# fabiocarrara/neural-ode-features

Measured on AMD Instinct MI355X. Metric: images/sec (fwd+adjoint) CIFAR-10 ODE-ResNet bs=128 at 1/2/4/8 GPU, higher is better.
Workload: dtype f32

## Files before the change

### include/node_hip.h

```cpp
#ifndef NODE_HIP_H
#define NODE_HIP_H

#include <stddef.h>
#include <stdint.h>

#ifdef __cplusplus
extern "C" {
#endif

#define NODE_ABI_VERSION 6

enum { NODE_METHOD_DOPRI5 = 0, NODE_METHOD_RK4 = 1 };

enum {
  NODE_OK = 0,
  NODE_ERR_NULL = -1,
  NODE_ERR_SHAPE = -2,
  NODE_ERR_UNSUPPORTED = -3,
  NODE_ERR_WORKSPACE = -4,
  NODE_ERR_MAX_STEPS = -5,
  NODE_ERR_NONFINITE = -6,
  NODE_ERR_DT_UNDERFLOW = -7,
  NODE_ERR_HIP = -8,
  NODE_ERR_ARG = -9
// ... 217 lines not shown
  const float* b1_c2_w;
  const float* b1_ds_w;
  const float* b2_n1_w;
  const float* b2_n1_b;
  const float* b2_c1_w;
  const float* b2_n2_w;
  const float* b2_n2_b;
  const float* b2_c2_w;
  const float* b2_ds_w;
} node_stem_params;
typedef struct node_stem_grads {
  float* conv0_w; float* conv0_b;
  float* b1_n1_w; float* b1_n1_b; float* b1_c1_w; float* b1_n2_w; float* b1_n2_b; float* b1_c2_w; float* b1_ds_w;
  float* b2_n1_w; float* b2_n1_b; float* b2_c1_w; float* b2_n2_w; float* b2_n2_b; float* b2_c2_w; float* b2_ds_w;
} node_stem_grads;
size_t node_stem_workspace_bytes(const node_stem_shape* shape);
int node_stem_fwd(const node_stem_shape* shape, const node_stem_params* params, const float* x, float* out,
                  void* ws, size_t ws_bytes, void* stream);
int node_stem_bwd(const node_stem_shape* shape, const node_stem_params* params, const float* x, const float* grad_out,
                  const node_stem_grads* grads, void* ws, size_t ws_bytes, void* stream);
int node_stem_bwd_dx(const node_stem_shape* shape, const node_stem_params* params, const float* x, const float* grad_out,
                     const node_stem_grads* grads, float* d_x, void* ws, size_t ws_bytes, void* stream);
size_t node_stem_conv0_dgrad_workspace_bytes(const node_stem_shape* shape);
int node_stem_conv0_dgrad(const node_stem_shape* shape, const float* w0, const float* dy, float* d_x,
                          void* ws, size_t ws_bytes, void* stream);

typedef struct node_conv_geom {
  int32_t n, cin, cout, x_h, x_w, k, stride, pad;
} node_conv_geom;
size_t node_stem_conv_workspace_bytes(const node_conv_geom* g);
int node_stem_conv(const node_conv_geom* g, int what, const float* x, const float* w, const float* dy, float* result,
                   void* ws, size_t ws_bytes, void* stream);

typedef struct node_trunk_shape {
  int32_t n, channels, h, w, blocks;
  float eps;
} node_trunk_shape;
typedef struct node_trunk_block {
  const float* n1_w;
  const float* n1_b;
  const float* c1_w;
  const float* n2_w;
  const float* n2_b;
  const float* c2_w;
} node_trunk_block;
typedef struct node_trunk_block_grads {
  float* n1_w; float* n1_b; float* c1_w; float* n2_w; float* n2_b; float* c2_w;
} node_trunk_block_grads;
size_t node_trunk_workspace_bytes(const node_trunk_shape* shape, int keep_for_backward);
int node_trunk_fwd(const node_trunk_shape* shape, const node_trunk_block* blocks, const float* x, float* out, float* taps,
                   int keep_for_backward, void* ws, size_t ws_bytes, void* stream);
int node_trunk_bwd(const node_trunk_shape* shape, const node_trunk_block* blocks, const float* grad_out,
                   const node_trunk_block_grads* grads, float* d_x, void* ws, size_t ws_bytes, void* stream);

size_t node_retrieval_workspace_bytes(int nq, int nd, int d);
int node_retrieval_ap(int nq, int nd, int d, const float* q, const float* x, const int32_t* q_labels, const int32_t* x_labels,
                      int k, double* ap, double* ap_k, void* ws, size_t ws_bytes, void* stream);
int node_rank_ap(int nq, int nd, const float* scores, const int32_t* q_labels, const int32_t* x_labels, int k, double* ap,
                 double* ap_k, void* ws, size_t ws_bytes, void* stream);

typedef struct { int32_t fold; int32_t cls; float c; } node_svm_problem;
typedef struct { int32_t iterations; int32_t converged; double grad_ratio; } node_svm_result;
size_t node_svm_workspace_bytes(int n, int d, int p);
int node_svm_fit(int n, int d, int p, const float* x, const int32_t* labels, const int32_t* row_fold,
                 const node_svm_problem* problems, double eps, int max_iter, float* weights, node_svm_result* results, void* ws,
                 size_t ws_bytes, void* stream);
// ... 55 lines not shown
```

### neural-ode-features_amd/_lib.py

```python
from __future__ import annotations

import ctypes as C
import os

HERE = os.path.dirname(os.path.abspath(__file__))
LIB_PATH = os.path.join(HERE, 'csrc', 'libnode_hip.so')
LIB_DIAG_PATH = os.path.join(HERE, 'csrc', 'libnode_hip_diag.so')

NODE_ABI_VERSION = 6
METHOD_DOPRI5, METHOD_RK4 = 0, 1
METHODS = {'dopri5': METHOD_DOPRI5, 'rk4': METHOD_RK4}

ERRORS = {
    0: 'NODE_OK', -1: 'NODE_ERR_NULL', -2: 'NODE_ERR_SHAPE', -3: 'NODE_ERR_UNSUPPORTED',
    -4: 'NODE_ERR_WORKSPACE', -5: 'NODE_ERR_MAX_STEPS', -6: 'NODE_ERR_NONFINITE',
    -7: 'NODE_ERR_DT_UNDERFLOW', -8: 'NODE_ERR_HIP', -9: 'NODE_ERR_ARG',
}

EXPORTS = [
    'node_abi_version', 'node_last_error', 'node_param_count', 'node_workspace_bytes', 'node_solve_is_resident',
    'node_describe_dims',
    'node_odefunc_fwd', 'node_odefunc_vjp', 'node_solve_fwd', 'node_solve_adjoint',
    'node_backprop_workspace_bytes', 'node_solve_backprop',
    'node_head_fwd', 'node_head_bwd', 'node_gn_relu_fwd', 'node_gn_relu_bwd',
    'node_sgd_step', 'node_adam_step', 'node_profile_begin', 'node_profile_end',
    'node_conv3x3_w4_workspace_bytes', 'node_conv3x3_w4', 'node_w4_split3', 'node_w4_pair_stats',
    'node_stem_workspace_bytes', 'node_stem_fwd', 'node_stem_bwd', 'node_stem_conv_workspace_bytes', 'node_stem_conv',
    'node_stem_bwd_dx', 'node_stem_conv0_dgrad_workspace_bytes', 'node_stem_conv0_dgrad', 'node_attack_step', 'node_attack_judge',
    'node_head_loss_scratch_bytes', 'node_head_loss_fwd', 'node_head_loss_bwd',
    'node_flat_workspace_bytes', 'node_flat_begin', 'node_flat_stage', 'node_flat_scalar', 'node_flat_initial_step',
    'node_flat_finish_step', 'node_flat_status_read',
    'node_retrieval_workspace_bytes', 'node_retrieval_ap', 'node_rank_ap',
    'node_svm_workspace_bytes', 'node_svm_fit', 'node_svm_cv_score',
    'node_augment_batch',
    'node_imgconv_workspace_bytes', 'node_imgconv_fwd', 'node_imgconv_bwd',
    'node_trunk_workspace_bytes', 'node_trunk_fwd', 'node_trunk_bwd',
]


class NodeShape(C.Structure):
    _fields_ = [('n', C.c_int32), ('c', C.c_int32), ('h', C.c_int32), ('w', C.c_int32),
                ('groups', C.c_int32), ('eps', C.c_float)]


class NodeParams(C.Structure):
    _fields_ = [(k, C.c_void_p) for k in (
        'norm1_w', 'norm1_b', 'conv1_w', 'conv1_b', 'norm2_w', 'norm2_b',
        'conv2_w', 'conv2_b', 'norm3_w', 'norm3_b')]


WGRAD_KERNELS = ('W2_8', 'W2_4', 'W_8_8', 'W_16_2', 'W_4_4', 'T_8_8', 'T_16_4', 'T_7_7', 'T_4_4', 'P')
CONV_KERNELS = ('DIRECT_64', 'DIRECT_128', 'DIRECT_256', 'W1_64', 'W1_128', 'W1_256', 'W2_128')


class NodeDimsInfo(C.Structure):
    _fields_ = [(k, C.c_int32) for k in (
        'wgrad_kernel', 'conv_kernel', 'wino', 'bm', 's', 'csplit', 'mtiles', 'ntile', 'small', 'tiny', 'wino4', 'w4q',
        'wgrad_wino', 'wut', 'rb', 'nbands', 'nsplit', 'wgrad_pair')]


# ... 43 lines not shown

class NodeAdamTensor(C.Structure):
    _fields_ = [('param', C.c_void_p), ('grad', C.c_void_p), ('exp_avg', C.c_void_p), ('exp_avg_sq', C.c_void_p),
                ('step', C.c_void_p), ('n', C.c_size_t)]


STEM_PARAM_FIELDS = ('conv0_w', 'conv0_b', 'b1_n1_w', 'b1_n1_b', 'b1_c1_w', 'b1_n2_w', 'b1_n2_b', 'b1_c2_w', 'b1_ds_w',
                     'b2_n1_w', 'b2_n1_b', 'b2_c1_w', 'b2_n2_w', 'b2_n2_b', 'b2_c2_w', 'b2_ds_w')


class NodeStemShape(C.Structure):
    _fields_ = [('n', C.c_int32), ('in_ch', C.c_int32), ('h', C.c_int32), ('w', C.c_int32), ('filters', C.c_int32),
                ('eps', C.c_float)]


class NodeStemParams(C.Structure):
    _fields_ = [(k, C.c_void_p) for k in STEM_PARAM_FIELDS]


TRUNK_BLOCK_FIELDS = ('n1_w', 'n1_b', 'c1_w', 'n2_w', 'n2_b', 'c2_w')


class NodeTrunkShape(C.Structure):
    _fields_ = [('n', C.c_int32), ('channels', C.c_int32), ('h', C.c_int32), ('w', C.c_int32), ('blocks', C.c_int32),
                ('eps', C.c_float)]


class NodeTrunkBlock(C.Structure):
    _fields_ = [(k, C.c_void_p) for k in TRUNK_BLOCK_FIELDS]


class NodeConvGeom(C.Structure):
    _fields_ = [(k, C.c_int32) for k in ('n', 'cin', 'cout', 'x_h', 'x_w', 'k', 'stride', 'pad')]


REDUCE_MEAN, REDUCE_SUM = 0, 1


class NodeHeadLoss(C.Structure):
    _fields_ = [('n', C.c_int32), ('c', C.c_int32), ('classes', C.c_int32), ('reduction', C.c_int32),
                ('pooled', C.c_void_p), ('weight', C.c_void_p), ('bias', C.c_void_p), ('target', C.c_void_p),
                ('logits', C.c_void_p), ('loss', C.c_void_p), ('stat', C.c_void_p), ('scratch', C.c_void_p)]


class NodeHeadLossGrad(C.Structure):
    _fields_ = [(k, C.c_void_p) for k in ('grad_loss', 'grad_logits', 'd_logits', 'd_pooled', 'd_weight', 'd_bias')]


class NodeFlatSeg(C.Structure):
    _fields_ = [('y', C.c_void_p), ('y1', C.c_void_p), ('k', C.c_void_p * 7), ('n', C.c_size_t)]


class NodeFlatSolve(C.Structure):
    _fields_ = [('nseg', C.c_int32), ('has_scalar', C.c_int32), ('seg', NodeFlatSeg * 3), ('rtol', C.c_float), ('atol', C.c_float),
                ('tsign', C.c_float), ('n_targets', C.c_int32), ('ws', C.c_void_p), ('ws_bytes', C.c_size_t)]


class NodeFlatStatus(C.Structure):
    _fields_ = [('done', C.c_int32), ('status', C.c_int32), ('steps', C.c_int32), ('accepted', C.c_int32), ('rejected', C.c_int32),
                ('t', C.c_double), ('dt', C.c_double), ('first_dt', C.c_double), ('scalar', C.c_float)]


FLAT_F0, FLAT_PROBE = -1, -2

AUG_CROP, AUG_JITTER, AUG_FLIP, AUG_NORM = 1, 2, 4, 8

# ... 75 lines not shown
    lib.node_head_fwd.argtypes = [P(NodeShape), vp, vp, vp, vp, vp, vp, vp]
    lib.node_head_bwd.restype = i32
    lib.node_head_bwd.argtypes = [P(NodeShape), vp, vp, vp, vp, vp, vp, vp, vp, vp, vp]
    lib.node_gn_relu_fwd.restype = i32
    lib.node_gn_relu_fwd.argtypes = [P(NodeShape), vp, vp, vp, i32, vp, vp, vp]
    lib.node_gn_relu_bwd.restype = i32
    lib.node_gn_relu_bwd.argtypes = [P(NodeShape), vp, vp, vp, vp, i32, vp, vp, vp, vp, vp]
    lib.node_sgd_step.restype = i32
    lib.node_sgd_step.argtypes = [P(NodeSgdTensor), i32, f32, f32, f32, f32, vp, vp]
    lib.node_adam_step.restype = i32
    lib.node_adam_step.argtypes = [P(NodeAdamTensor), i32, f32, f32, f32, f32, f32, f32, vp, vp]
    lib.node_profile_begin.restype = i32
    lib.node_profile_begin.argtypes = []
    lib.node_profile_end.restype = i32
    lib.node_profile_end.argtypes = [P(NodeProfile)]
    lib.node_conv3x3_w4_workspace_bytes.restype = sz
    lib.node_conv3x3_w4_workspace_bytes.argtypes = [P(NodeShape)]
    lib.node_w4_pair_stats.restype = i32
    lib.node_w4_pair_stats.argtypes = [P(C.c_int32)]
    lib.node_conv3x3_w4.restype = i32
    lib.node_conv3x3_w4.argtypes = [P(NodeShape), vp, i32, vp, vp, vp, sz, vp]
    lib.node_w4_split3.restype = i32
    lib.node_w4_split3.argtypes = [vp, vp, sz, vp]
    lib.node_stem_workspace_bytes.restype = sz
    lib.node_stem_workspace_bytes.argtypes = [P(NodeStemShape)]
    lib.node_stem_fwd.restype = i32
    lib.node_stem_fwd.argtypes = [P(NodeStemShape), P(NodeStemParams), vp, vp, vp, sz, vp]
    lib.node_stem_bwd.restype = i32
    lib.node_stem_bwd.argtypes = [P(NodeStemShape), P(NodeStemParams), vp, vp, P(NodeStemParams), vp, sz, vp]
    lib.node_stem_conv_workspace_bytes.restype = sz
    lib.node_stem_conv_workspace_bytes.argtypes = [P(NodeConvGeom)]
    lib.node_stem_conv.restype = i32
    lib.node_stem_conv.argtypes = [P(NodeConvGeom), i32, vp, vp, vp, vp, vp, sz, vp]
    lib.node_stem_bwd_dx.restype = i32
    lib.node_stem_bwd_dx.argtypes = [P(NodeStemShape), P(NodeStemParams), vp, vp, P(NodeStemParams), vp, vp, sz, vp]
    lib.node_stem_conv0_dgrad_workspace_bytes.restype = sz
    lib.node_stem_conv0_dgrad_workspace_bytes.argtypes = [P(NodeStemShape)]
    lib.node_stem_conv0_dgrad.restype = i32
    lib.node_stem_conv0_dgrad.argtypes = [P(NodeStemShape), vp, vp, vp, vp, sz, vp]
    lib.node_attack_step.restype = i32
    lib.node_attack_step.argtypes = [P(NodeAttack), vp, vp, vp, vp, vp, vp]
    lib.node_attack_judge.restype = i32
    lib.node_attack_judge.argtypes = [P(NodeAttack), i32, vp, vp, vp, vp, i32, i32, P(NodeAttackRecord), vp]
    lib.node_head_loss_scratch_bytes.restype = sz
    lib.node_head_loss_scratch_bytes.argtypes = [i32]
    lib.node_head_loss_fwd.restype = i32
    lib.node_head_loss_fwd.argtypes = [P(NodeHeadLoss), vp]
    lib.node_head_loss_bwd.restype = i32
    lib.node_head_loss_bwd.argtypes = [P(NodeHeadLoss), P(NodeHeadLossGrad), vp]
    lib.node_flat_workspace_bytes.restype = sz
    lib.node_flat_workspace_bytes.argtypes = [i32]
    lib.node_flat_begin.restype = i32
    lib.node_flat_begin.argtypes = [P(NodeFlatSolve), C.c_double, P(C.c_double), C.c_double, i32, vp]
    lib.node_flat_stage.restype = i32
    lib.node_flat_stage.argtypes = [P(NodeFlatSolve), i32, i32, P(C.c_void_p), vp, vp]
    lib.node_flat_scalar.restype = i32
    lib.node_flat_scalar.argtypes = [P(NodeFlatSolve), i32, vp, f32, i32, vp]
    lib.node_flat_initial_step.restype = i32
    lib.node_flat_initial_step.argtypes = [P(NodeFlatSolve), i32, vp]
    lib.node_flat_finish_step.restype = i32
    lib.node_flat_finish_step.argtypes = [P(NodeFlatSolve), i32, vp, vp]
    lib.node_flat_status_read.restype = i32
    lib.node_flat_status_read.argtypes = [P(NodeFlatSolve), P(NodeFlatStatus), vp]
    lib.node_retrieval_workspace_bytes.restype = sz
    lib.node_retrieval_workspace_bytes.argtypes = [i32, i32, i32]
    lib.node_retrieval_ap.restype = i32
# ... 34 lines not shown
```

### neural-ode-features_amd/csrc/kernels_stem.hip

```cpp
#include "stem.h"
#include <type_traits>

namespace node {

namespace {

typedef float f32x16 __attribute__((ext_vector_type(16)));
typedef __bf16 bf16x8 __attribute__((ext_vector_type(8)));
typedef __bf16 bf16x2 __attribute__((ext_vector_type(2)));
typedef float f32x2 __attribute__((ext_vector_type(2)));
typedef unsigned u32x4 __attribute__((ext_vector_type(4)));

__device__ __forceinline__ void split3(float x, bf16_t& h, bf16_t& m, bf16_t& l) {
  const __bf16 bh = (__bf16)x;
  const float r = x - (float)bh;
  const __bf16 bm = (__bf16)r;
  const float r2 = r - (float)bm;
  const __bf16 bl = (__bf16)r2;
  h = __builtin_bit_cast(bf16_t, bh);
  m = __builtin_bit_cast(bf16_t, bm);
  l = __builtin_bit_cast(bf16_t, bl);
}
__device__ __forceinline__ void split8(const float4& p, const float4& q, u32x4& hh, u32x4& mm, u32x4& ll) {
  const f32x2 v[4] = {{p.x, p.y}, {p.z, p.w}, {q.x, q.y}, {q.z, q.w}};
// ... 723 lines not shown
  __syncthreads();
  const float inv_m = 1.f / (float)(a.cpg * HW);
  const int q8 = CB >> 3;
  for (int idx = t; idx < HW * q8; idx += 256) {
    const int px = idx / q8, q = idx - px * q8;
    float v[8];
#pragma unroll
    for (int k = 0; k < 8; ++k) {
      const int cc = 8 * q + k, g = cc / a.cpg;
      const float xh = txh[px * CB + cc], dy = tdy[px * CB + cc];
      v[k] = grstd[g] * (dy * a.gamma[c0 + cc] - (gs1[g] + xh * gs2[g]) * inv_m);
    }
    const size_t o = ((size_t)n * HW + px) * C + c0 + 8 * q;
    if constexpr (SKIP) {
      const float4 k0 = *reinterpret_cast<const float4*>(a.skip + o), k1 = *reinterpret_cast<const float4*>(a.skip + o + 4);
      v[0] += k0.x; v[1] += k0.y; v[2] += k0.z; v[3] += k0.w;
      v[4] += k1.x; v[5] += k1.y; v[6] += k1.z; v[7] += k1.w;
    }
    const float4 p0 = make_float4(v[0], v[1], v[2], v[3]), p1 = make_float4(v[4], v[5], v[6], v[7]);
    if (a.dh) {
      *reinterpret_cast<float4*>(a.dh + o) = p0;
      *reinterpret_cast<float4*>(a.dh + o + 4) = p1;
    }
    if (a.dh3) {
      u32x4 hh, mm, ll;
      split8(p0, p1, hh, mm, ll);
      *reinterpret_cast<u32x4*>(a.dh3 + o) = hh;
      *reinterpret_cast<u32x4*>(a.dh3 + o + a.dh_plane) = mm;
      *reinterpret_cast<u32x4*>(a.dh3 + o + 2 * a.dh_plane) = ll;
    }
  }
}

__global__ __launch_bounds__(256) void k_stem_from_nchw(const float* __restrict__ src, float* __restrict__ dst, bf16_t* __restrict__ dst3,
                                                        size_t plane, int C, int HW) {
  __shared__ float tile[64][65];
  const int t = threadIdx.x;
  const int npb = (HW + 63) / 64, ncb = C / 64;
  const int n = blockIdx.x / (npb * ncb), rem = blockIdx.x - n * npb * ncb, cb = rem / npb, pb = rem - cb * npb;
  const int c0 = cb * 64, p0 = pb * 64;
  for (int idx = t; idx < 64 * 64; idx += 256) {
    const int cc = idx >> 6, pp = idx & 63;
    tile[cc][pp] = p0 + pp < HW ? src[((size_t)n * C + c0 + cc) * HW + p0 + pp] : 0.f;
  }
  __syncthreads();
  for (int idx = t; idx < 64 * 8; idx += 256) {
    const int pp = idx >> 3, q = idx & 7;
    if (p0 + pp >= HW) continue;
    float v[8];
#pragma unroll
    for (int k = 0; k < 8; ++k) v[k] = tile[8 * q + k][pp];
    const size_t o = ((size_t)n * HW + p0 + pp) * C + c0 + 8 * q;
    const float4 a0 = make_float4(v[0], v[1], v[2], v[3]), a1 = make_float4(v[4], v[5], v[6], v[7]);
    if (dst) {
      *reinterpret_cast<float4*>(dst + o) = a0;
      *reinterpret_cast<float4*>(dst + o + 4) = a1;
    }
    if (dst3) {
      u32x4 hh, mm, ll;
      split8(a0, a1, hh, mm, ll);
      *reinterpret_cast<u32x4*>(dst3 + o) = hh;
      *reinterpret_cast<u32x4*>(dst3 + o + plane) = mm;
      *reinterpret_cast<u32x4*>(dst3 + o + 2 * plane) = ll;
    }
  }
}
// ... 158 lines not shown
    else STEM_WG(1, false, STEM_RING_D)
  } else {
    if (taps == 9 && a.dy23) STEM_WG(3, true, 1)
    else if (taps == 9) STEM_WG(3, false, 1)
    else STEM_WG(1, false, 1)
  }
#undef STEM_WG
}

void launch_stem_conv0_fwd(const float* x, const float* w0t, const float* bias, float* h0, int N, int Cin, int H, int W, hipStream_t s) {
  const int rows = N * (H - 2) * (W - 2);
  hipLaunchKernelGGL(k_stem_conv0_fwd, dim3((rows + 127) / 128), dim3(256), 0, s, x, w0t, bias, h0, N, Cin, H, W);
}
void launch_stem_conv0_wgrad(const float* x, const float* dh0, float* slab, int N, int Cin, int H, int W, int nsplit, int rows_per_split,
                             hipStream_t s) {
  hipLaunchKernelGGL(k_stem_conv0_wgrad, dim3(nsplit), dim3(256), 0, s, x, dh0, slab, N, Cin, H, W, rows_per_split);
}
void launch_stem_conv0_dgrad(const float* dh0, const float* w0, float* dx, int N, int Cin, int H, int W, hipStream_t s) {
  const int tx = (W + DG_TW - 1) / DG_TW, ty = (H + DG_TH - 1) / DG_TH;
  hipLaunchKernelGGL(k_stem_conv0_dgrad, dim3((unsigned)(N * tx * ty)), dim3(256), 0, s, dh0, w0, dx, Cin, H, W, tx, ty);
}

int stem_gn_cb(int HW, int C, int cpg) {
  const size_t budget = 150 * 1024;
  int cb = 8;
  while (cb < cpg) cb *= 2;
  if (cb > C || cb > 128 || (size_t)HW * cb * 2 * sizeof(float) > budget) return 0;
  while (cb * 2 <= C && cb * 2 <= 128 && (size_t)HW * cb * 4 * sizeof(float) <= budget) cb *= 2;
  static const int cap = env_int("NODE_TUNE_STEM_GNCB", -1);
  while (cap > 0 && cb > cap && cb / 2 >= cpg && cb / 2 >= 8) cb /= 2;
  if (C % cb != 0 || cb % cpg != 0) return 0;
  return cb;
}
void launch_stem_gn_fwd(const SGnArgs& a, hipStream_t s) {
  static bool attr[MAX_DEVICES] = {};
  allow_full_lds(reinterpret_cast<const void*>(k_stem_gn_fwd), attr);
  hipLaunchKernelGGL(k_stem_gn_fwd, dim3(a.N * (a.C / a.CB)), dim3(256), ((size_t)a.HW * a.CB + 512) * sizeof(float), s, a);
}
void launch_stem_gn_bwd(const SGnArgs& a, hipStream_t s) {
  const dim3 grid(a.N * (a.C / a.CB));
  const size_t lds = ((size_t)2 * a.HW * a.CB + 1024) * sizeof(float);
  if (a.skip) {
    static bool attr[MAX_DEVICES] = {};
    allow_full_lds(reinterpret_cast<const void*>(k_stem_gn_bwd<true>), attr);
    hipLaunchKernelGGL(k_stem_gn_bwd<true>, grid, dim3(256), lds, s, a);
  } else {
    static bool attr[MAX_DEVICES] = {};
    allow_full_lds(reinterpret_cast<const void*>(k_stem_gn_bwd<false>), attr);
    hipLaunchKernelGGL(k_stem_gn_bwd<false>, grid, dim3(256), lds, s, a);
  }
}

void launch_stem_prep(const SPrepArgs& a0, hipStream_t s) {
  SPrepArgs a = a0;
  unsigned at = 0;
  for (int i = 0; i < 6; ++i) {
    a.blk0[i] = at;
    if (i < a.njobs) at += (unsigned)(((size_t)a.job[i].taps * a.job[i].Cout * a.job[i].Cin + 255) / 256);
  }
  a.blk0[6] = at; at += (28 * 64 + 255) / 256;
  a.blk0[7] = at; at += (unsigned)(((size_t)a.nzero * 3 * 4096 + 255) / 256);
  a.blk0[8] = at;
  hipLaunchKernelGGL(k_stem_prep, dim3(at), dim3(256), 0, s, a);
}
void launch_stem_from_nchw(const float* src, float* dst_nhwc, bf16_t* dst3, size_t plane, int N, int C, int HW, hipStream_t s) {
  hipLaunchKernelGGL(k_stem_from_nchw, dim3(N * (C / 64) * ((HW + 63) / 64)), dim3(256), 0, s, src, dst_nhwc, dst3, plane, C, HW);
}
void launch_stem_split(const float* src, bf16_t* dst3, size_t plane, size_t n, hipStream_t s) {
  hipLaunchKernelGGL(k_stem_split, dim3((unsigned)((n / 8 + 255) / 256)), dim3(256), 0, s, src, dst3, plane, n / 8);
}
void launch_stem_to_nchw(const float* src_nhwc, float* dst, int N, int C, int HW, hipStream_t s) {
  hipLaunchKernelGGL(k_stem_to_nchw, dim3(N * (C / 64) * ((HW + 63) / 64)), dim3(256), 0, s, src_nhwc, dst, C, HW);
}
void launch_stem_reduce(const SReduceArgs& a0, hipStream_t s) {
  SReduceArgs a = a0;
  unsigned at = 0;
  for (int i = 0; i < a.njobs; ++i) {
    const SReduceJob& j = a.job[i];
    a.blk0[i] = at;
    at += (unsigned)(j.kind == 0 ? j.Co * j.taps : j.kind == 1 ? 64 : (2 * j.Co + 31) / 32);
  }
  a.blk0[a.njobs] = at;
  if (at == 0) return;
  hipLaunchKernelGGL(k_stem_reduce, dim3(at), dim3(256), 0, s, a);
}

}
```

### neural-ode-features_amd/csrc/stem.h

```cpp
#pragma once
#include "node_internal.h"

namespace node {

typedef unsigned short bf16_t;

struct SConvArgs {
  const bf16_t* in;
  size_t in_plane;
  int zero_row;
  const bf16_t* w;
  size_t w_plane;
  float* out;
  const float* res;
  const float* bias;
  int accumulate;
  const bf16_t* w2;
  size_t w2_plane;
  float* out2;
  const bf16_t* in2;
  int N, IH, IW;
  int OH, OW;
  int Cin, Cout;
  int KH, KW, sshift, pad;
// ... 14 lines not shown
  const bf16_t* in;
  size_t in_plane;
  int zero_row;
  float* slab;
  float* slab2;
  int N, IH, IW, OH, OW, Cin, Cout, KH, KW, stride, pad;
  int nsplit, rows_per_split;
};
void launch_stem_wgrad(const SWgradArgs& a, hipStream_t s);

void launch_stem_conv0_fwd(const float* x, const float* w0t , const float* bias, float* h0 , int N, int Cin,
                           int H, int W, hipStream_t s);
void launch_stem_conv0_wgrad(const float* x, const float* dh0, float* slab, int N, int Cin, int H, int W, int nsplit,
                             int rows_per_split, hipStream_t s);
void launch_stem_conv0_dgrad(const float* dh0, const float* w0, float* dx, int N, int Cin, int H, int W, hipStream_t s);

struct SGnArgs {
  const float* h;
  const float* gamma;
  const float* beta;
  float* stats;
  bf16_t* a3;
  size_t a_plane;
  const float* da;
  float* dh;
  bf16_t* dh3;
  size_t dh_plane;
  float* gpart;
  const float* skip;
  int N, HW, C, cpg, CB;
  float eps;
};
int stem_gn_cb(int HW, int C, int cpg);
void launch_stem_gn_fwd(const SGnArgs& a, hipStream_t s);
void launch_stem_gn_bwd(const SGnArgs& a, hipStream_t s);

struct SPrepJob { const float* w; bf16_t* wf; bf16_t* wd; int Cout, Cin, taps; };
struct SPrepArgs {
  SPrepJob job[6];
  int njobs;
  const float* w0; float* w0t; int k0;
  bf16_t* zero[10]; size_t zero_plane[10]; int zero_c[10]; int nzero;
  unsigned blk0[9];
};
void launch_stem_prep(const SPrepArgs& a, hipStream_t s);
void launch_stem_from_nchw(const float* src, float* dst_nhwc, bf16_t* dst3, size_t plane, int N, int C, int HW, hipStream_t s);
void launch_stem_to_nchw(const float* src_nhwc, float* dst, int N, int C, int HW, hipStream_t s);
void launch_stem_split(const float* src, bf16_t* dst3, size_t plane, size_t n , hipStream_t s);
struct SReduceJob { const float* slab; float* out; float* out2; int kind, ns, Co, Ci, taps; };
struct SReduceArgs { SReduceJob job[12]; int njobs; unsigned blk0[13]; };
void launch_stem_reduce(const SReduceArgs& a, hipStream_t s);

}
```

### neural-ode-features_amd/csrc/stem_api.hip

```cpp
#include "host_common.h"
#include "stem.h"
#include "stem_plan.h"
#include "wino4.h"
#include <cstring>

using namespace node;

namespace {

inline int down2(int h) { return (h - 1) / 2 + 1; }

struct StemPlan {
  int N, Cin0, H, W, F;
  int H0, W0, H1, W1, H2, W2, R0, R1, R2;
  float eps;
  float* w0t;
  Filt c1, c2, d1, c3, c4, d2;
  float *h0, *h1, *s1, *x1, *h3, *s2, *outn;
  Trip a0, a1, a2, a3;
  float* stats[4];
  float *da3, *da2, *da1, *da0, *dh0;
  Trip g3, dh3t, dx1t, dh1t;
  float* gpart[4];
  Wg w4, w3, w2, w1, w0;
// ... 451 lines not shown
  const int XHW = g->x_h * g->x_w, YHW = p.YH * p.YW;
  SPrepArgs pa;
  memset(&pa, 0, sizeof(pa));
  if (what != 2) { pa.job[0] = {w, p.f.wf, p.f.wd, g->cout, g->cin, g->k * g->k}; pa.njobs = 1; }
  pa.zero[0] = p.xin.p + (size_t)p.xin.rows * p.xin.C; pa.zero_plane[0] = p.xin.plane; pa.zero_c[0] = p.xin.C;
  pa.zero[1] = p.dyt.p + (size_t)p.dyt.rows * p.dyt.C; pa.zero_plane[1] = p.dyt.plane; pa.zero_c[1] = p.dyt.C;
  pa.nzero = 2;
  launch_stem_prep(pa, st);
  if (what == 0) {
    launch_stem_from_nchw(x, nullptr, p.xin.p, p.xin.plane, g->n, g->cin, XHW, st);
    launch_stem_conv(conv_fwd_args(p.xin, p.f, p.resn, g->n, g->x_h, g->x_w, p.YH, p.YW, g->k, g->stride, g->pad), st);
    launch_stem_to_nchw(p.resn, result, g->n, g->cout, YHW, st);
  } else if (what == 1) {
    launch_stem_from_nchw(dy, nullptr, p.dyt.p, p.dyt.plane, g->n, g->cout, YHW, st);
    SConvArgs c = conv_dgrad_args(p.dyt, p.f, p.resn, g->n, p.YH, p.YW, g->x_h, g->x_w, g->k, g->stride, g->pad);
    if (g->k == 1 && g->stride == 2) {
      if (hipMemsetAsync(p.resn, 0, (size_t)g->n * XHW * g->cin * sizeof(float), st) != hipSuccess) return fail(NODE_ERR_HIP, "memset failed");
    }
    launch_stem_conv(c, st);
    launch_stem_to_nchw(p.resn, result, g->n, g->cin, XHW, st);
  } else {
    launch_stem_from_nchw(x, nullptr, p.xin.p, p.xin.plane, g->n, g->cin, XHW, st);
    launch_stem_from_nchw(dy, nullptr, p.dyt.p, p.dyt.plane, g->n, g->cout, YHW, st);
    launch_stem_wgrad(wgrad_args(p.dyt, nullptr, p.xin, p.wg, g->n, g->x_h, g->x_w, p.YH, p.YW, g->cin, g->cout, g->k, g->stride, g->pad), st);
    SReduceArgs ra;
    memset(&ra, 0, sizeof(ra));
    ra.job[0] = {p.wg.slab, result, nullptr, 0, p.wg.nsplit, g->cout, g->cin, g->k * g->k};
    ra.njobs = 1;
    launch_stem_reduce(ra, st);
  }
  return launch_ok("node_stem_conv");
}

}
```

Baseline: 29410.

## Add register-resident one-block-per-sample GroupNorm kernels for the stem

Adds GroupNorm+ReLU forward and backward kernels that keep each sample's activations in registers, launching one large block per sample and reducing over channel octets with shuffles plus shared memory. A streaming backward variant handles large spatial sizes. The default env setting enables only the backward path (bit 1); the forward register path is off unless the tuning variable is set. The aim is to avoid staging whole channel blocks in LDS and to remove multiple global passes, at the cost of fewer, larger blocks. A standalone node_stem_gn test API and a join kernel are also added.

```diff
diff --git a/include/node_hip.h b/include/node_hip.h
--- a/include/node_hip.h
+++ b/include/node_hip.h
@@ -273,6 +273,15 @@
 int node_stem_conv(const node_conv_geom* g, int what, const float* x, const float* w, const float* dy, float* result,
                    void* ws, size_t ws_bytes, void* stream);
 
+typedef struct node_gn_geom {
+  int32_t n, c, h, w;
+  float eps;
+} node_gn_geom;
+size_t node_stem_gn_workspace_bytes(const node_gn_geom* g);
+int node_stem_gn(const node_gn_geom* g, int what, const float* x, const float* gamma, const float* beta, const float* dy,
+                 const float* skip, float* result, float* result3, float* stats, float* dgamma, float* dbeta,
+                 void* ws, size_t ws_bytes, void* stream);
+
 typedef struct node_trunk_shape {
   int32_t n, channels, h, w, blocks;
   float eps;
diff --git a/neural-ode-features_amd/_lib.py b/neural-ode-features_amd/_lib.py
--- a/neural-ode-features_amd/_lib.py
+++ b/neural-ode-features_amd/_lib.py
@@ -26,6 +26,7 @@
     'node_sgd_step', 'node_adam_step', 'node_profile_begin', 'node_profile_end',
     'node_conv3x3_w4_workspace_bytes', 'node_conv3x3_w4', 'node_w4_split3', 'node_w4_pair_stats',
     'node_stem_workspace_bytes', 'node_stem_fwd', 'node_stem_bwd', 'node_stem_conv_workspace_bytes', 'node_stem_conv',
+    'node_stem_gn_workspace_bytes', 'node_stem_gn',
     'node_stem_bwd_dx', 'node_stem_conv0_dgrad_workspace_bytes', 'node_stem_conv0_dgrad', 'node_attack_step', 'node_attack_judge',
     'node_head_loss_scratch_bytes', 'node_head_loss_fwd', 'node_head_loss_bwd',
     'node_flat_workspace_bytes', 'node_flat_begin', 'node_flat_stage', 'node_flat_scalar', 'node_flat_initial_step',
@@ -135,6 +136,10 @@
 
 class NodeConvGeom(C.Structure):
     _fields_ = [(k, C.c_int32) for k in ('n', 'cin', 'cout', 'x_h', 'x_w', 'k', 'stride', 'pad')]
+
+
+class NodeGnGeom(C.Structure):
+    _fields_ = [('n', C.c_int32), ('c', C.c_int32), ('h', C.c_int32), ('w', C.c_int32), ('eps', C.c_float)]
 
 
 REDUCE_MEAN, REDUCE_SUM = 0, 1
@@ -276,6 +281,10 @@
     lib.node_stem_conv_workspace_bytes.argtypes = [P(NodeConvGeom)]
     lib.node_stem_conv.restype = i32
     lib.node_stem_conv.argtypes = [P(NodeConvGeom), i32, vp, vp, vp, vp, vp, sz, vp]
+    lib.node_stem_gn_workspace_bytes.restype = sz
+    lib.node_stem_gn_workspace_bytes.argtypes = [P(NodeGnGeom)]
+    lib.node_stem_gn.restype = i32
+    lib.node_stem_gn.argtypes = [P(NodeGnGeom), i32, vp, vp, vp, vp, vp, vp, vp, vp, vp, vp, vp, sz, vp]
     lib.node_stem_bwd_dx.restype = i32
     lib.node_stem_bwd_dx.argtypes = [P(NodeStemShape), P(NodeStemParams), vp, vp, P(NodeStemParams), vp, vp, sz, vp]
     lib.node_stem_conv0_dgrad_workspace_bytes.restype = sz
diff --git a/neural-ode-features_amd/csrc/kernels_stem.hip b/neural-ode-features_amd/csrc/kernels_stem.hip
--- a/neural-ode-features_amd/csrc/kernels_stem.hip
+++ b/neural-ode-features_amd/csrc/kernels_stem.hip
@@ -779,6 +779,325 @@
   }
 }
 
+constexpr int GNR_TF = 1024, GNR_TB = 512;
+constexpr int GNR_NPF = 8, GNR_NPB = 8;
+constexpr int GNR_MAXOQ = 256;
+constexpr int GNR_DEFAULT = 1;
+
+template <int T, int NV>
+__device__ __forceinline__ void octet_sums(float (&v)[NV], float* red, float* tot, int OQ, int oshift, int t) {
+  const int lane = t & 63, w = t >> 6;
+#pragma unroll
+  for (int off = 32; off >= 1; off >>= 1)
+    if (off >= OQ) {
+#pragma unroll
+      for (int k = 0; k < NV; ++k) v[k] += __shfl_xor(v[k], off, 64);
+    }
+  if (lane < OQ) {
+#pragma unroll
+    for (int k = 0; k < NV; k += 4) *reinterpret_cast<float4*>(red + (w * 64 + lane) * NV + k) = make_float4(v[k], v[k + 1], v[k + 2], v[k + 3]);
+  }
+  __syncthreads();
+  const int ncov = OQ <= 64 ? T / 64 : T >> oshift, wstep = OQ <= 64 ? 1 : OQ >> 6;
+  for (int j = t; j < OQ * NV; j += T) {
+    const int o = j / NV, k = j - o * NV, w0 = OQ <= 64 ? 0 : o >> 6;
+    float s = 0.f;
+    for (int i = 0; i < ncov; ++i) s += red[((w0 + i * wstep) * 64 + (o & 63)) * NV + k];
+    tot[j] = s;
+  }
+  __syncthreads();
+  const int o = t & (OQ - 1);
+#pragma unroll
+  for (int k = 0; k < NV; k += 4) {
+    const float4 p = *reinterpret_cast<const float4*>(tot + o * NV + k);
+    v[k] = p.x; v[k + 1] = p.y; v[k + 2] = p.z; v[k + 3] = p.w;
+  }
+}
+__device__ __forceinline__ void group_combine(float (&s)[8], int cpg) {
+  if (cpg >= 2) {
+#pragma unroll
+    for (int k = 0; k < 8; k += 2) s[k] = s[k + 1] = s[k] + s[k + 1];
+  }
+  if (cpg >= 4) {
+#pragma unroll
+    for (int k = 0; k < 8; k += 4) s[k] = s[k + 1] = s[k + 2] = s[k + 3] = s[k] + s[k + 2];
+  }
+  if (cpg >= 8) {
+    float g = s[0] + s[4];
+    for (int off = 1; off * 8 < cpg; off <<= 1) g += __shfl_xor(g, off, 64);
+#pragma unroll
+    for (int k = 0; k < 8; ++k) s[k] = g;
+  }
+}
+#define GNR_F8(p0, p1) {(p0).x, (p0).y, (p0).z, (p0).w, (p1).x, (p1).y, (p1).z, (p1).w}
+
+template <bool SKIP>
+__device__ __forceinline__ void gnr_store(const SGnArgs& a, size_t at, float (&r)[8]) {
+  if constexpr (SKIP) {
+    const float4 k0 = *reinterpret_cast<const float4*>(a.skip + at), k1 = *reinterpret_cast<const float4*>(a.skip + at + 4);
+    r[0] += k0.x; r[1] += k0.y; r[2] += k0.z; r[3] += k0.w;
+    r[4] += k1.x; r[5] += k1.y; r[6] += k1.z; r[7] += k1.w;
+  }
+  const float4 p0 = make_float4(r[0], r[1], r[2], r[3]), p1 = make_float4(r[4], r[5], r[6], r[7]);
+  if (a.dh) {
+    *reinterpret_cast<float4*>(a.dh + at) = p0;
+    *reinterpret_cast<float4*>(a.dh + at + 4) = p1;
+  }
+  if (a.dh3) {
+    u32x4 hh, mm, ll;
+    split8(p0, p1, hh, mm, ll);
+    *reinterpret_cast<u32x4*>(a.dh3 + at) = hh;
+    *reinterpret_cast<u32x4*>(a.dh3 + at + a.dh_plane) = mm;
+    *reinterpret_cast<u32x4*>(a.dh3 + at + 2 * a.dh_plane) = ll;
+  }
+}
+
+template <int NP>
+__global__ __launch_bounds__(GNR_TF) void k_stem_gn_fwd_reg(const SGnArgs a) {
+  __shared__ __align__(16) float red[GNR_TF * 8];
+  __shared__ __align__(16) float tot[GNR_MAXOQ * 8];
+  const int t = threadIdx.x, n = blockIdx.x, C = a.C, HW = a.HW;
+  const int OQ = C >> 3, oshift = __ffs(OQ) - 1, o = t & (OQ - 1), slot = t >> oshift, PS = GNR_TF >> oshift;
+  const int cshift = __ffs(a.cpg) - 1;
+  const size_t sample = (size_t)n * HW * C;
+  const unsigned tq = 8u * t;
+  float4 v[NP][2];
+#pragma unroll
+  for (int i = 0; i < NP; ++i) {
+    const int px = slot + i * PS;
+    if (px < HW) {
+      const float* p = a.h + (sample + (size_t)i * (8 * GNR_TF)) + tq;
+      v[i][0] = *reinterpret_cast<const float4*>(p);
+      v[i][1] = *reinterpret_cast<const float4*>(p + 4);
+    } else {
+      v[i][0] = v[i][1] = make_float4(0.f, 0.f, 0.f, 0.f);
+    }
+  }
+  float s[8] = {0.f, 0.f, 0.f, 0.f, 0.f, 0.f, 0.f, 0.f};
+#pragma unroll
+  for (int i = 0; i < NP; ++i) {
+    const float x[8] = GNR_F8(v[i][0], v[i][1]);
+#pragma unroll
+    for (int k = 0; k < 8; ++k) s[k] += x[k];
+  }
+  group_combine(s, a.cpg);
+  octet_sums<GNR_TF, 8>(s, red, tot, OQ, oshift, t);
+  const float inv_m = 1.f / (float)(a.cpg * HW);
+  float mean[8], q[8];
+#pragma unroll
+  for (int k = 0; k < 8; ++k) { mean[k] = s[k] * inv_m; q[k] = 0.f; }
+#pragma unroll
+  for (int i = 0; i < NP; ++i) {
+    const float x[8] = GNR_F8(v[i][0], v[i][1]);
+    const bool on = slot + i * PS < HW;
+#pragma unroll
+    for (int k = 0; k < 8; ++k) {
+      const float d = on ? x[k] - mean[k] : 0.f;
+      q[k] += d * d;
+    }
+  }
+  group_combine(q, a.cpg);
+  octet_sums<GNR_TF, 8>(q, red, tot, OQ, oshift, t);
+  float rstd[8];
+#pragma unroll
+  for (int k = 0; k < 8; ++k) rstd[k] = rsqrtf(q[k] * inv_m + a.eps);
+  if (slot == 0) {
+#pragma unroll
+    for (int k = 0; k < 8; ++k) {
+      const int c = 8 * o + k;
+      if ((c & (a.cpg - 1)) == 0) {
+        float* st = a.stats + ((size_t)n * (C >> cshift) + (c >> cshift)) * 2;
+        st[0] = mean[k];
+        st[1] = rstd[k];
+      }
+    }
+  }
+  float gam[8], bet[8];
+#pragma unroll
+  for (int k = 0; k < 8; ++k) { gam[k] = a.gamma[8 * o + k]; bet[k] = a.beta[8 * o + k]; }
+#pragma unroll
+  for (int i = 0; i < NP; ++i) {
+    const int px = slot + i * PS;
+    if (px < HW) {
+      float x[8] = GNR_F8(v[i][0], v[i][1]);
+#pragma unroll
+      for (int k = 0; k < 8; ++k) {
+        const float y = (x[k] - mean[k]) * rstd[k] * gam[k] + bet[k];
+        x[k] = fmaxf(y, 0.f);
+      }
+      u32x4 hh, mm, ll;
+      split8(make_float4(x[0], x[1], x[2], x[3]), make_float4(x[4], x[5], x[6], x[7]), hh, mm, ll);
+      bf16_t* dst = a.a3 + (sample + (size_t)i * (8 * GNR_TF)) + tq;
+      *reinterpret_cast<u32x4*>(dst) = hh;
+      *reinterpret_cast<u32x4*>(dst + a.a_plane) = mm;
+      *reinterpret_cast<u32x4*>(dst + 2 * a.a_plane) = ll;
+    }
+  }
+}
+
+template <int NP, bool SKIP>
+__global__ __launch_bounds__(GNR_TB) void k_stem_gn_bwd_reg(const SGnArgs a) {
+  __shared__ __align__(16) float red[GNR_TB * 16];
+  __shared__ __align__(16) float tot[GNR_MAXOQ * 16];
+  const int t = threadIdx.x, n = blockIdx.x, C = a.C, HW = a.HW;
+  const int OQ = C >> 3, oshift = __ffs(OQ) - 1, o = t & (OQ - 1), slot = t >> oshift, PS = GNR_TB >> oshift;
+  const int cshift = __ffs(a.cpg) - 1;
+  const size_t sample = (size_t)n * HW * C;
+  const unsigned tq = 8u * t;
+  float4 x[NP][2], d[NP][2];
+#pragma unroll
+  for (int i = 0; i < NP; ++i) {
+    if (slot + i * PS < HW) {
+      const size_t at = (sample + (size_t)i * (8 * GNR_TB)) + tq;
+      x[i][0] = *reinterpret_cast<const float4*>(a.h + at);
+      x[i][1] = *reinterpret_cast<const float4*>(a.h + at + 4);
+      d[i][0] = *reinterpret_cast<const float4*>(a.da + at);
+      d[i][1] = *reinterpret_cast<const float4*>(a.da + at + 4);
+    } else {
+      x[i][0] = x[i][1] = d[i][0] = d[i][1] = make_float4(0.f, 0.f, 0.f, 0.f);
+    }
+  }
+  float mean[8], rstd[8], gam[8], bet[8];
+#pragma unroll
+  for (int k = 0; k < 8; ++k) {
+    const int c = 8 * o + k;
+    const float* st = a.stats + ((size_t)n * (C >> cshift) + (c >> cshift)) * 2;
+    mean[k] = st[0]; rstd[k] = st[1];
+    gam[k] = a.gamma[c]; bet[k] = a.beta[c];
+  }
+  float acc[16];
+#pragma unroll
+  for (int k = 0; k < 16; ++k) acc[k] = 0.f;
+#pragma unroll
+  for (int i = 0; i < NP; ++i) {
+    const float xv[8] = GNR_F8(x[i][0], x[i][1]);
+    float dv[8] = GNR_F8(d[i][0], d[i][1]), xh[8];
+#pragma unroll
+    for (int k = 0; k < 8; ++k) {
+      xh[k] = (xv[k] - mean[k]) * rstd[k];
+      const float y = xh[k] * gam[k] + bet[k];
+      dv[k] = y > 0.f ? dv[k] : 0.f;
+      acc[k] += dv[k];
+      acc[8 + k] += dv[k] * xh[k];
+    }
+    x[i][0] = make_float4(xh[0], xh[1], xh[2], xh[3]);
+    x[i][1] = make_float4(xh[4], xh[5], xh[6], xh[7]);
+    d[i][0] = make_float4(dv[0], dv[1], dv[2], dv[3]);
+    d[i][1] = make_float4(dv[4], dv[5], dv[6], dv[7]);
+  }
+  octet_sums<GNR_TB, 16>(acc, red, tot, OQ, oshift, t);
+  if (slot == 0) {
+    float* gp = a.gpart + (size_t)n * 2 * C + 8 * o;
+#pragma unroll
+    for (int k = 0; k < 8; ++k) {
+      gp[k] = acc[8 + k];
+      gp[C + k] = acc[k];
+    }
+  }
+  float s1[8], s2[8];
+#pragma unroll
+  for (int k = 0; k < 8; ++k) { s1[k] = acc[k] * gam[k]; s2[k] = acc[8 + k] * gam[k]; }
+  group_combine(s1, a.cpg);
+  group_combine(s2, a.cpg);
+  const float inv_m = 1.f / (float)(a.cpg * HW);
+#pragma unroll
+  for (int i = 0; i < NP; ++i) {
+    if (slot + i * PS < HW) {
+      const size_t at = (sample + (size_t)i * (8 * GNR_TB)) + tq;
+      const float xh[8] = GNR_F8(x[i][0], x[i][1]), dv[8] = GNR_F8(d[i][0], d[i][1]);
+      float r[8];
+#pragma unroll
+      for (int k = 0; k < 8; ++k) r[k] = rstd[k] * (dv[k] * gam[k] - (s1[k] + xh[k] * s2[k]) * inv_m);
+      gnr_store<SKIP>(a, at, r);
+    }
+  }
+}
+
+template <bool SKIP>
+__global__ __launch_bounds__(GNR_TF) void k_stem_gn_bwd_stream(const SGnArgs a) {
+  __shared__ __align__(16) float red[GNR_TF * 8];
+  __shared__ __align__(16) float tot[GNR_MAXOQ * 8];
+  const int t = threadIdx.x, n = blockIdx.x, C = a.C, HW = a.HW;
+  const int OQ = C >> 3, oshift = __ffs(OQ) - 1, o = t & (OQ - 1), slot = t >> oshift, PS = GNR_TF >> oshift;
+  const int cshift = __ffs(a.cpg) - 1;
+  const size_t sample = (size_t)n * HW * C;
+  const unsigned tq = 8u * t;
+  float mean[8], rstd[8], gam[8], bet[8];
+#pragma unroll
+  for (int k = 0; k < 8; ++k) {
+    const int c = 8 * o + k;
+    const float* st = a.stats + ((size_t)n * (C >> cshift) + (c >> cshift)) * 2;
+    mean[k] = st[0]; rstd[k] = st[1];
+    gam[k] = a.gamma[c]; bet[k] = a.beta[c];
+  }
+  float sA[8], sB[8];
+#pragma unroll
+  for (int k = 0; k < 8; ++k) sA[k] = sB[k] = 0.f;
+#pragma unroll 4
+  for (int px = slot; px < HW; px += PS) {
+    const size_t at = (sample + (size_t)(px - slot) * C) + tq;
+    const float4 x0 = *reinterpret_cast<const float4*>(a.h + at), x1 = *reinterpret_cast<const float4*>(a.h + at + 4);
+    const float4 d0 = *reinterpret_cast<const float4*>(a.da + at), d1 = *reinterpret_cast<const float4*>(a.da + at + 4);
+    const float xv[8] = GNR_F8(x0, x1), dv[8] = GNR_F8(d0, d1);
+#pragma unroll
+    for (int k = 0; k < 8; ++k) {
+      const float xh = (xv[k] - mean[k]) * rstd[k];
+      const float y = xh * gam[k] + bet[k];
+      const float dy = y > 0.f ? dv[k] : 0.f;
+      sA[k] += dy;
+      sB[k] += dy * xh;
+    }
+  }
+  octet_sums<GNR_TF, 8>(sA, red, tot, OQ, oshift, t);
+  octet_sums<GNR_TF, 8>(sB, red, tot, OQ, oshift, t);
+  if (slot == 0) {
+    float* gp = a.gpart + (size_t)n * 2 * C + 8 * o;
+#pragma unroll
+    for (int k = 0; k < 8; ++k) {
+      gp[k] = sB[k];
+      gp[C + k] = sA[k];
+    }
+  }
+  float s1[8], s2[8];
+#pragma unroll
+  for (int k = 0; k < 8; ++k) { s1[k] = sA[k] * gam[k]; s2[k] = sB[k] * gam[k]; }
+  group_combine(s1, a.cpg);
+  group_combine(s2, a.cpg);
+  const float inv_m = 1.f / (float)(a.cpg * HW);
+  const int last = slot < HW ? (HW - 1 - slot) / PS : -1;
+#pragma unroll 2
+  for (int j = last; j >= 0; --j) {
+    const size_t at = (sample + (size_t)j * PS * C) + tq;
+    const float4 x0 = *reinterpret_cast<const float4*>(a.h + at), x1 = *reinterpret_cast<const float4*>(a.h + at + 4);
+    const float4 d0 = *reinterpret_cast<const float4*>(a.da + at), d1 = *reinterpret_cast<const float4*>(a.da + at + 4);
+    const float xv[8] = GNR_F8(x0, x1), dv[8] = GNR_F8(d0, d1);
+    float r[8];
+#pragma unroll
+    for (int k = 0; k < 8; ++k) {
+      const float xh = (xv[k] - mean[k]) * rstd[k];
+      const float y = xh * gam[k] + bet[k];
+      const float dy = y > 0.f ? dv[k] : 0.f;
+      r[k] = rstd[k] * (dy * gam[k] - (s1[k] + xh * s2[k]) * inv_m);
+    }
+    gnr_store<SKIP>(a, at, r);
+  }
+}
+
+__global__ __launch_bounds__(256) void k_stem_join(const bf16_t* __restrict__ src3, size_t plane, float* __restrict__ dst, size_t n8) {
+  const size_t i = (size_t)blockIdx.x * 256 + threadIdx.x;
+  if (i >= n8) return;
+  const u32x4 hh = *reinterpret_cast<const u32x4*>(src3 + 8 * i), mm = *reinterpret_cast<const u32x4*>(src3 + 8 * i + plane),
+              ll = *reinterpret_cast<const u32x4*>(src3 + 8 * i + 2 * plane);
+  float r[8];
+#pragma unroll
+  for (int k = 0; k < 4; ++k) {
+    r[2 * k] = (bf16_f((bf16_t)(hh[k] & 0xffffu)) + bf16_f((bf16_t)(mm[k] & 0xffffu))) + bf16_f((bf16_t)(ll[k] & 0xffffu));
+    r[2 * k + 1] = (bf16_f((bf16_t)(hh[k] >> 16)) + bf16_f((bf16_t)(mm[k] >> 16))) + bf16_f((bf16_t)(ll[k] >> 16));
+  }
+  reinterpret_cast<float4*>(dst)[2 * i] = make_float4(r[0], r[1], r[2], r[3]);
+  reinterpret_cast<float4*>(dst)[2 * i + 1] = make_float4(r[4], r[5], r[6], r[7]);
+}
+
 __global__ __launch_bounds__(256) void k_stem_from_nchw(const float* __restrict__ src, float* __restrict__ dst, bf16_t* __restrict__ dst3,
                                                         size_t plane, int C, int HW) {
   __shared__ float tile[64][65];
@@ -1003,12 +1322,55 @@
   if (C % cb != 0 || cb % cpg != 0) return 0;
   return cb;
 }
+bool stem_gn_reg(int HW, int C, int cpg, bool forward) {
+  if ((env_int("NODE_TUNE_STEM_GN_REG", GNR_DEFAULT) & (forward ? 2 : 1)) == 0) return false;
+  if (HW <= 0 || C < 8 || C % 8 != 0 || cpg <= 0 || C % cpg != 0) return false;
+  const int oq = C / 8;
+  if ((oq & (oq - 1)) != 0 || oq > GNR_MAXOQ || (cpg & (cpg - 1)) != 0 || cpg > 512) return false;
+  return (HW + GNR_TF / oq - 1) / (GNR_TF / oq) <= GNR_NPF;
+}
+static int gnr_chain(int HW, int threads, int C) {
+  const int ps = threads / (C / 8), np = (HW + ps - 1) / ps;
+  int c = 1;
+  while (c < np) c *= 2;
+  return c;
+}
 void launch_stem_gn_fwd(const SGnArgs& a, hipStream_t s) {
+  if (stem_gn_reg(a.HW, a.C, a.cpg, true)) {
+    switch (gnr_chain(a.HW, GNR_TF, a.C)) {
+      case 1: hipLaunchKernelGGL(k_stem_gn_fwd_reg<1>, dim3(a.N), dim3(GNR_TF), 0, s, a); break;
+      case 2: hipLaunchKernelGGL(k_stem_gn_fwd_reg<2>, dim3(a.N), dim3(GNR_TF), 0, s, a); break;
+      case 4: hipLaunchKernelGGL(k_stem_gn_fwd_reg<4>, dim3(a.N), dim3(GNR_TF), 0, s, a); break;
+      default: hipLaunchKernelGGL(k_stem_gn_fwd_reg<8>, dim3(a.N), dim3(GNR_TF), 0, s, a); break;
+    }
+    return;
+  }
   static bool attr[MAX_DEVICES] = {};
   allow_full_lds(reinterpret_cast<const void*>(k_stem_gn_fwd), attr);
   hipLaunchKernelGGL(k_stem_gn_fwd, dim3(a.N * (a.C / a.CB)), dim3(256), ((size_t)a.HW * a.CB + 512) * sizeof(float), s, a);
 }
 void launch_stem_gn_bwd(const SGnArgs& a, hipStream_t s) {
+  if (stem_gn_reg(a.HW, a.C, a.cpg, false)) {
+#define GNR_BWD(NP)                                                                                         \
+    if (a.skip) hipLaunchKernelGGL((k_stem_gn_bwd_reg<NP, true>), dim3(a.N), dim3(GNR_TB), 0, s, a);        \
+    else hipLaunchKernelGGL((k_stem_gn_bwd_reg<NP, false>), dim3(a.N), dim3(GNR_TB), 0, s, a);              \
+    break;
+    static_assert(GNR_NPB == 8, "the chains instantiated below");
+    const int np = gnr_chain(a.HW, GNR_TB, a.C);
+    if (np > GNR_NPB) {
+      if (a.skip) hipLaunchKernelGGL(k_stem_gn_bwd_stream<true>, dim3(a.N), dim3(GNR_TF), 0, s, a);
+      else hipLaunchKernelGGL(k_stem_gn_bwd_stream<false>, dim3(a.N), dim3(GNR_TF), 0, s, a);
+      return;
+    }
+    switch (np) {
+      case 1: GNR_BWD(1)
+      case 2: GNR_BWD(2)
+      case 4: GNR_BWD(4)
+      default: GNR_BWD(8)
+    }
+#undef GNR_BWD
+    return;
+  }
   const dim3 grid(a.N * (a.C / a.CB));
   const size_t lds = ((size_t)2 * a.HW * a.CB + 1024) * sizeof(float);
   if (a.skip) {
@@ -1034,6 +1396,9 @@
   a.blk0[8] = at;
   hipLaunchKernelGGL(k_stem_prep, dim3(at), dim3(256), 0, s, a);
 }
+void launch_stem_join(const bf16_t* src3, size_t plane, float* dst, size_t n, hipStream_t s) {
+  hipLaunchKernelGGL(k_stem_join, dim3((unsigned)((n / 8 + 255) / 256)), dim3(256), 0, s, src3, plane, dst, n / 8);
+}
 void launch_stem_from_nchw(const float* src, float* dst_nhwc, bf16_t* dst3, size_t plane, int N, int C, int HW, hipStream_t s) {
   hipLaunchKernelGGL(k_stem_from_nchw, dim3(N * (C / 64) * ((HW + 63) / 64)), dim3(256), 0, s, src, dst_nhwc, dst3, plane, C, HW);
 }
diff --git a/neural-ode-features_amd/csrc/stem.h b/neural-ode-features_amd/csrc/stem.h
--- a/neural-ode-features_amd/csrc/stem.h
+++ b/neural-ode-features_amd/csrc/stem.h
@@ -70,6 +70,7 @@
   float eps;
 };
 int stem_gn_cb(int HW, int C, int cpg);
+bool stem_gn_reg(int HW, int C, int cpg, bool forward);
 void launch_stem_gn_fwd(const SGnArgs& a, hipStream_t s);
 void launch_stem_gn_bwd(const SGnArgs& a, hipStream_t s);
 
@@ -85,6 +86,7 @@
 void launch_stem_from_nchw(const float* src, float* dst_nhwc, bf16_t* dst3, size_t plane, int N, int C, int HW, hipStream_t s);
 void launch_stem_to_nchw(const float* src_nhwc, float* dst, int N, int C, int HW, hipStream_t s);
 void launch_stem_split(const float* src, bf16_t* dst3, size_t plane, size_t n , hipStream_t s);
+void launch_stem_join(const bf16_t* src3, size_t plane, float* dst, size_t n , hipStream_t s);
 struct SReduceJob { const float* slab; float* out; float* out2; int kind, ns, Co, Ci, taps; };
 struct SReduceArgs { SReduceJob job[12]; int njobs; unsigned blk0[13]; };
 void launch_stem_reduce(const SReduceArgs& a, hipStream_t s);
diff --git a/neural-ode-features_amd/csrc/stem_api.hip b/neural-ode-features_amd/csrc/stem_api.hip
--- a/neural-ode-features_amd/csrc/stem_api.hip
+++ b/neural-ode-features_amd/csrc/stem_api.hip
@@ -507,4 +507,91 @@
   return launch_ok("node_stem_conv");
 }
 
-}
+namespace {
+struct GnPlan {
+  int HW, G;
+  float *xn, *dan, *skipn, *dhn, *resn, *stats, *gpart;
+  Trip a3, dh3;
+  size_t bytes;
+};
+GnPlan make_gn(const node_gn_geom* g, void* base) {
+  GnPlan p;
+  Bump b(base);
+  p.HW = g->h * g->w;
+  p.G = g->c < 32 ? g->c : 32;
+  const size_t elems = (size_t)g->n * p.HW * g->c;
+  p.xn = b.take<float>(elems);
+  p.dan = b.take<float>(elems);
+  p.skipn = b.take<float>(elems);
+  p.dhn = b.take<float>(elems);
+  p.resn = b.take<float>(elems);
+  p.stats = b.take<float>((size_t)g->n * p.G * 2);
+  p.gpart = b.take<float>((size_t)g->n * 2 * g->c);
+  p.a3 = take_trip(b, g->n * p.HW, g->c);
+  p.dh3 = take_trip(b, g->n * p.HW, g->c);
+  p.bytes = b.off + 256;
+  return p;
+}
+int check_gn(const node_gn_geom* g) {
+  if (!g) return fail(NODE_ERR_NULL, "geometry is NULL");
+  if (g->n <= 0 || g->c <= 0 || g->h <= 0 || g->w <= 0) return fail(NODE_ERR_SHAPE, "bad geometry");
+  if (g->c % 64 != 0) return fail(NODE_ERR_UNSUPPORTED, "channels must be a multiple of 64 (got %d)", g->c);
+  if ((size_t)g->n * g->h * g->w * g->c >= ((size_t)1 << 31)) return fail(NODE_ERR_UNSUPPORTED, "stem tensors must stay under 2^31 elements");
+  if (stem_gn_cb(g->h * g->w, g->c, g->c / 32) == 0)
+    return fail(NODE_ERR_UNSUPPORTED, "%d pixels x %d channels: no GroupNorm channel block fits the LDS", g->h * g->w, g->c);
+  return NODE_OK;
+}
+}
+
+size_t node_stem_gn_workspace_bytes(const node_gn_geom* g) {
+  if (check_gn(g) != NODE_OK) return 0;
+  return make_gn(g, nullptr).bytes;
+}
+
+int node_stem_gn(const node_gn_geom* g, int what, const float* x, const float* gamma, const float* beta, const float* dy, const float* skip,
+                 float* result, float* result3, float* stats, float* dgamma, float* dbeta, void* ws, size_t ws_bytes, void* stream) {
+  int rc = check_gn(g);
+  if (rc != NODE_OK) return rc;
+  if (what != 0 && what != 1) return fail(NODE_ERR_ARG, "what must be 0 (forward) or 1 (backward)");
+  if (!x || !gamma || !beta || !ws) return fail(NODE_ERR_NULL, "a required pointer is NULL");
+  if (what == 0 && (!result || !stats)) return fail(NODE_ERR_NULL, "the forward needs result and stats");
+  if (what == 1 && (!dy || !dgamma || !dbeta || (!result && !result3))) return fail(NODE_ERR_NULL, "the backward needs dy, dgamma, dbeta and a result");
+  if (((uintptr_t)ws) & 255) return fail(NODE_ERR_ARG, "workspace must be 256-byte aligned");
+  GnPlan p = make_gn(g, ws);
+  if (ws_bytes < p.bytes) return fail(NODE_ERR_WORKSPACE, "workspace too small");
+  hipStream_t st = (hipStream_t)stream;
+  const size_t elems = (size_t)g->n * p.HW * g->c;
+  launch_stem_from_nchw(x, p.xn, nullptr, 0, g->n, g->c, p.HW, st);
+  SGnArgs a = gn_args(p.xn, gamma, beta, what == 0 ? stats : p.stats, g->n, p.HW, g->c, g->eps);
+  a.a3 = p.a3.p; a.a_plane = p.a3.plane;
+  launch_stem_gn_fwd(a, st);
+  if ((rc = launch_ok("stem_gn_fwd")) != NODE_OK) return rc;
+  if (what == 0) {
+    launch_stem_join(p.a3.p, p.a3.plane, p.resn, elems, st);
+    launch_stem_to_nchw(p.resn, result, g->n, g->c, p.HW, st);
+    return launch_ok("node_stem_gn");
+  }
+  launch_stem_from_nchw(dy, p.dan, nullptr, 0, g->n, g->c, p.HW, st);
+  if (skip) launch_stem_from_nchw(skip, p.skipn, nullptr, 0, g->n, g->c, p.HW, st);
+  a.da = p.dan;
+  a.skip = skip ? p.skipn : nullptr;
+  a.dh = result ? p.dhn : nullptr;
+  a.dh3 = result3 ? p.dh3.p : nullptr;
+  a.dh_plane = p.dh3.plane;
+  a.gpart = p.gpart;
+  launch_stem_gn_bwd(a, st);
+  if ((rc = launch_ok("stem_gn_bwd")) != NODE_OK) return rc;
+  if (result) launch_stem_to_nchw(p.dhn, result, g->n, g->c, p.HW, st);
+  if (result3) {
+    launch_stem_join(p.dh3.p, p.dh3.plane, p.resn, elems, st);
+    launch_stem_to_nchw(p.resn, result3, g->n, g->c, p.HW, st);
+  }
+  SReduceArgs ra;
+  memset(&ra, 0, sizeof(ra));
+  ra.job[0] = {p.gpart, dgamma, dbeta, 2, g->n, g->c, 0, 0};
+  ra.njobs = 1;
+  launch_stem_reduce(ra, st);
+  return launch_ok("node_stem_gn");
+}
+
+}
```

Result: no change. 29680, median of 6 (+0.9%).
